# ErickRosete/tacorl

Hardware: AMD Instinct MI355X
Metric: offline grad-steps/sec (batch=256, 84x84 RGB) (higher is better)
Workload: dtype bf16; 1 GPU; tacorl actor-critic training_step, frozen LMP (BASELINE configs[1]); per_gpu_batch=256, global_batch=256, window=16, image=84x84x3, frames=fp32 CHW (reference batch schema), latent_plan=16, n_action_samples=4, phase=Q (epoch>=bc_epochs), action_decoder_loss=every step (reference behaviour), parallelism=dp1, hip_graph=True, losses_finite=True

## Files before the change

### include/tacorl_hip.h

```cpp
#ifndef TACORL_HIP_H
#define TACORL_HIP_H
#include <stddef.h>
#ifdef __cplusplus
extern "C" {
#endif

typedef void* tacorl_stream_t;

#define TACORL_MAXP 16
enum { TACORL_F32 = 0, TACORL_BF16 = 1 };
enum { TACORL_ACT_NONE = 0, TACORL_ACT_RELU = 1, TACORL_ACT_SILU = 2, TACORL_ACT_TANH = 3 };

int tacorl_hip_version(void);
int tacorl_hip_init(int device);
const char* tacorl_hip_last_error(void);
int tacorl_time_mark(unsigned long long* marks, int slot, tacorl_stream_t stream);
int tacorl_time_spin(unsigned long long* marks, int slot, long ticks, tacorl_stream_t stream);

int tacorl_linear_fwd(int nprob, const float* const* x, int ldx, const float* const* w,
                      const float* const* b, float* const* y, float* const* z, const int* M,
                      int K, int N, int act, int compute_dtype, tacorl_stream_t stream);
size_t tacorl_linear_add_fwd_ws_bytes(int nprob, const int* M, int K, int N);
int tacorl_linear_add_fwd(int nprob, const float* const* x, int ldx, const float* const* w,
                          const float* const* b, const float* const* addend, int ld_add, float* const* y,
// ... 294 lines not shown
                      float* dq1, float* dq2, float grad_scale, float* logs, tacorl_stream_t stream);
int tacorl_actor_head_bwd(const float* head, int ld_head, const float* eps, const float* logp,
                          const float* g_act1, const float* g_act2, int ld_g, const float* value,
                          int ld_value, const int* grip_idx, const float* log_alpha, float grad_scale,
                          float* d_head, int B, int Ac, int has_grip, float* logs, tacorl_stream_t stream);
int tacorl_tanh_normal_nll(const float* head, int ld_head, const float* target, int ld_target, int M, int Ac,
                           int has_grip, float grad_scale, float* d_head, float* loss_out, tacorl_stream_t stream);

size_t tacorl_cql_ws_bytes(int B);
int tacorl_cql_loss(const float* q1, const float* q2, float* dq1, float* dq2, const float* tq1,
                    const float* tq2, const float* logp_cur, const float* logp_nxt, const float* next_logp,
                    const float* reward, const float* done, const float* log_alpha,
                    const float* log_alpha_prime, int B, int n, int A, float discount, float reward_scale,
                    float temp, float cons_w, float gap, int deterministic_backup, float grad_scale,
                    float* g_log_alpha_prime, float* logs, void* ws, size_t ws_bytes, tacorl_stream_t stream);

size_t tacorl_adam_ws_bytes(long n);
int tacorl_adam_step(float* param, const float* grad, float* m, float* v, long n, float lr,
                     float max_norm, int* step_counter, float* target, float tau, void* ws,
                     size_t ws_bytes, tacorl_stream_t stream);
size_t tacorl_adam_batch_ws_bytes(int nb);
int tacorl_adam_step_batch(int nb, float* const* param, const float* const* grad, float* const* m,
                           float* const* v, const long* n, const float* lr, const float* max_norm,
                           int* const* step_counter, float* const* target, const float* tau, void* ws,
                           size_t ws_bytes, tacorl_stream_t stream);
int tacorl_adam_step_batch_mirror(int nb, float* const* param, const float* const* grad, float* const* m,
                                  float* const* v, const long* n, const float* lr, const float* max_norm,
                                  int* const* step_counter, float* const* target, const float* tau,
                                  void* const* mirror, void* const* target_mirror, void* ws, size_t ws_bytes,
                                  tacorl_stream_t stream);
// ... 14 lines not shown
```

### tacorl_amd/_lib.py

```python
import ctypes as C
import os

HERE = os.path.dirname(os.path.abspath(__file__))
LIB_PATH = os.environ.get("TACORL_HIP_LIB") or os.path.join(HERE, "lib", "libtacorl_hip.so")

F32, BF16 = 0, 1
ACT_NONE, ACT_RELU, ACT_SILU, ACT_TANH = 0, 1, 2, 3
MAXP = 16

LOG_SLOTS = [
    "alpha_loss", "alpha", "actor_loss", "bellman_q1_loss", "bellman_q2_loss", "conservative_q1_loss",
    "conservative_q2_loss", "q1_loss", "q2_loss", "alpha_prime", "alpha_prime_loss", "q1_data", "q1_random",
    "q1_policy", "q2_data", "q2_random", "q2_policy", "action_loss",
]

_p, _i, _l, _f, _sz = C.c_void_p, C.c_int, C.c_long, C.c_float, C.c_size_t
_SIGS = {
    "tacorl_hip_version": (_i, []),
    "tacorl_hip_init": (_i, [_i]),
    "tacorl_hip_last_error": (C.c_char_p, []),
    "tacorl_time_mark": (_i, [_p, _i, _p]),
    "tacorl_time_spin": (_i, [_p, _i, _l, _p]),
    "tacorl_linear_fwd": (_i, [_i, _p, _i, _p, _p, _p, _p, _p, _i, _i, _i, _i, _p]),
    "tacorl_linear_add_fwd_ws_bytes": (_sz, [_i, _p, _i, _i]),
# ... 106 lines not shown
    "tacorl_sample_transitions": (_i, [_p, _l, _p, _p, _i, _p, _l, _p, _p, _p, _p, _p, _p, _l, _l, _i, _i, _p, _p, _p, _p, _p, _p]),
    "tacorl_copy_cols": (_i, [_p, _i, _p, _i, _i, _i, _i, _i, _p]),
    "tacorl_copy_cols_batch": (_i, [_i, _p, _p, _p, _p, _p, _p, _p, _p, _p]),
    "tacorl_reduce_rows_mod": (_i, [_p, _i, _p, _i, _i, _i, _i, _p]),
    "tacorl_reduce_rows_mod_batch": (_i, [_i, _p, _i, _p, _i, _i, _i, _i, _p]),
    "tacorl_uniform_actions": (_i, [_p, _p, _i, _i, _i, _i, _p]),
    "tacorl_tanh_normal_sample": (_i, [_p, _i, _p, _p, _i, _p, _i, _p, _p, _i, _i, _i, _p]),
    "tacorl_tanh_normal_sample_batch": (_i, [_i, _p, _i, _p, _p, _p, _p, _i, _p, _p, _p, _i, _i, _p, _p, _i, _i, _i, _p]),
    "tacorl_alpha_loss": (_i, [_p, _i, _p, _f, _f, _p, _p, _p]),
    "tacorl_alpha_loss_step": (_i, [_p, _i, _p, _f, _p, _p, _p, _p, _f, _p, _p]),
    "tacorl_actor_qmin": (_i, [_p, _p, _p, _i, _p, _p, _p, _f, _p, _p]),
    "tacorl_actor_head_bwd": (_i, [_p, _i, _p, _p, _p, _p, _i, _p, _i, _p, _p, _f, _p, _i, _i, _i, _p, _p]),
    "tacorl_tanh_normal_nll": (_i, [_p, _i, _p, _i, _i, _i, _i, _f, _p, _p, _p]),
    "tacorl_cql_ws_bytes": (_sz, [_i]),
    "tacorl_cql_loss": (_i, [_p] * 13 + [_i, _i, _i, _f, _f, _f, _f, _f, _i, _f, _p, _p, _p, _sz, _p]),
    "tacorl_adam_ws_bytes": (_sz, [_l]),
    "tacorl_adam_step": (_i, [_p, _p, _p, _p, _l, _f, _f, _p, _p, _f, _p, _sz, _p]),
    "tacorl_adam_batch_ws_bytes": (_sz, [_i]),
    "tacorl_adam_step_batch": (_i, [_i, _p, _p, _p, _p, _p, _p, _p, _p, _p, _p, _p, _sz, _p]),
    "tacorl_adam_step_batch_mirror": (_i, [_i, _p, _p, _p, _p, _p, _p, _p, _p, _p, _p, _p, _p, _p, _sz, _p]),
    "tacorl_cem_supported": (_i, [_i, _i, _i, _i, _i, _i]),
    "tacorl_cem_ws_bytes": (_sz, [_i, _i, _i, _i, _i, _i, _i]),
    "tacorl_cem_refine": (_i, [_i, _i, _p, _p, _p, _p, _p, _p, _i, _i, _i, _i, _i, _i, _i, _f, _f, _f, _i, _i, _p, _p, _p, _p, _p,
                               _p, _sz, _p]),
}

_lib = None


class TacorlHipError(RuntimeError):
# ... 71 lines not shown
```

### tacorl_amd/csrc/dense_ops.hip

```cpp
#include <stdio.h>
#include <stdlib.h>
#include <string.h>

#include <type_traits>

#include "../../include/tacorl_hip.h"
#include "enc_bwd_fused.h"
#include "mlp_fused.h"
#include "functors.h"

static thread_local char g_err[256] = "";
#define FAIL(code, ...)                        \
  do {                                         \
    snprintf(g_err, sizeof(g_err), __VA_ARGS__); \
    return (code);                             \
  } while (0)
#define CHECK(x)            \
  do {                      \
    int _r = (x);           \
    if (_r != TACORL_OK) return _r; \
  } while (0)

extern "C" const char* tacorl_hip_last_error(void) { return g_err; }
extern "C" int tacorl_hip_version(void) { return 1; }
// ... 998 lines not shown
  for (int p = 0; p < nprob; p++) {
    long z1[MLP_MAXL], y1[MLP_MAXL];
    tacorl_mlp_act_layout(M[p], L, dims, acts, z1, y1);
    const int b = (lean && mlp_big_prob_ok(M[p], L, dims, acts)) ? 1 : 0, q = n[b]++;
    gm[b][q] = p;
    xs[b][q] = x ? x[p] : nullptr; ps[b][q] = params[p]; pb[b][q] = params_bf16[p]; as[b][q] = act[p]; Ms[b][q] = M[p];
    for (int l = 0; l < L; l++) {
      if (b) { ybf[q * MF_MAXL + l] = y1[l]; sbf[q * MF_MAXL + l] = z1[l]; }
      else {
        zo[q * MF_MAXL + l] = z1[l];
        yo[q * MF_MAXL + l] = (lean && l + 1 < L && z1[l] >= 0) ? -1 : y1[l];
      }
    }
    if (b) yout[q] = y1[L - 1];
  }
  if (n[1]) {
    const int rc = mlp_big_fwd(n[1], xs[1], ldx, ps[1], pb[1], as[1], Ms[1], L, dims, acts, ybf, sbf, yout, wo, bo, (hipStream_t)stream, gather, gm[1]);
    if (rc != TACORL_OK) FAIL(rc, "mlp_fwd_fused: many-row launch failed (%d)", rc);
  }
  if (n[0]) {
    const int rc = mlp_fused_fwd(n[0], xs[0], ldx, ps[0], pb[0], as[0], Ms[0], L, dims, acts, zo, yo, wo, bo, (hipStream_t)stream, gather, gm[0]);
    if (rc != TACORL_OK) FAIL(rc, "mlp_fwd_fused: launch failed (%d)", rc);
  }
  return TACORL_OK;
}
extern "C" int tacorl_mlp_fwd_fused(int nprob, const float* const* x, int ldx, const float* const* params,
                                    const void* const* params_bf16, float* const* act, const int* M, int L,
                                    const int* dims, const int* acts, int lean, tacorl_stream_t stream) {
  return mlp_fwd_fused_impl(nprob, x, ldx, params, params_bf16, act, M, L, dims, acts, lean, stream, nullptr);
}
// ... 310 lines not shown
```

### tacorl_amd/csrc/mlp_fused.h

```cpp
#pragma once
#include <hip/hip_runtime.h>

#define MF_MAXP 8
#define MF_MAXL 4
#define MF_MAXSEG 4

struct MlpXGather {
  const float* ptr[MF_MAXP][MF_MAXSEG];
  int ld[MF_MAXP][MF_MAXSEG], c0[MF_MAXP][MF_MAXSEG], mod[MF_MAXP][MF_MAXSEG];
  int nseg[MF_MAXP];
  float* xw[MF_MAXP];
};

bool mlp_fused_fwd_ok(int nprob, int L, const int* dims, int ldx);
int mlp_fused_fwd(int nprob, const float* const* x, int ldx, const float* const* params, const void* const* params_bf16,
                  float* const* act,
                  const int* M, int L, const int* dims, const int* acts, const long* zoff, const long* yoff,
                  const long* woff, const long* boff, hipStream_t st, const MlpXGather* gather = nullptr,
                  const int* gmap = nullptr);

bool mlp_fused_bwd_ok(int nprob, int L, const int* dims, int ldo, int ldd);
size_t mlp_fused_wt_elems(int L, const int* dims, long* wtoff);
int mlp_fused_bwd(int nprob, const float* const* params, const float* const* act, const float* const* d_out, int ldo,
                  float* const* dz, float* const* d_x, int ldd, void* const* wt, const int* M, int L, const int* dims,
// ... 1 lines not shown
bool prep_deferring();
int prep_defer_bf16(const float* src, void* dst, long count, hipStream_t st);

bool mlp_fused_wgrad_ok(int nprob, int L, const int* dims);
size_t mlp_fused_wgrad_slab_floats(int nprob, const int* M, int L, const int* dims);
int mlp_fused_wgrad(int nprob, const float* const* x, int ldx, const float* const* act, const float* const* d_out, int ldo,
                    const float* const* dz, float* const* grads, float* slab, const int* M, int L, const int* dims,
                    const long* yoff, const long* dzoff, const long* woff, const long* boff, int accumulate, hipStream_t st,
                    const int* acts = nullptr);

bool mlp_big_prob_ok(int M, int L, const int* dims, const int* acts);
int mlp_big_fwd(int nprob, const float* const* x, int ldx, const float* const* params, const void* const* params_bf16,
                float* const* act, const int* M, int L, const int* dims, const int* acts, const long* ybf, const long* sbf,
                const long* yout, const long* woff, const long* boff, hipStream_t st, const MlpXGather* gather = nullptr,
                const int* gmap = nullptr);
int mlp_big_bwd(int nprob, const float* const* act, const float* const* d_out, int ldo, float* const* dz, float* const* d_x,
                int ldd, void* const* wt, const int* M, int L, const int* dims, const long* sbf, const long* dzoff,
                hipStream_t st);
size_t mlp_big_wgrad_slab_floats(int nprob, const int* M, int L, const int* dims);
size_t mlp_big_xb_bytes(int M);
int mlp_fused_wgrad_big(int nprob, const float* const* x, int ldx, const float* const* act, const float* const* d_out, int ldo,
                        const float* const* dz, float* const* grads, float* slab, void* const* xb, const int* M, int L,
                        const int* dims, const long* ybf, const long* dzoff, const long* woff, const long* boff, int accumulate,
                        hipStream_t st, size_t slab_floats);
```

### tacorl_amd/csrc/mlp_fused.hip

```cpp
#include "mlp_fused.h"

#include <stdlib.h>

#include "common.h"

namespace {

constexpr int BMF = 32;
constexpr int MTF = BMF / 16;
constexpr int XP = 272;
constexpr int MAXD = 256;
constexpr int MF_NT = 1024, MF_CW = MAXD / (MF_NT / 64), MF_NTW = MF_CW / 16;

struct MlpXSeg { const float* p; int ld, c0, mod, pad; };
struct MlpFwdArgs {
  MlpXSeg seg[MF_MAXP][MF_MAXSEG];
  int nseg[MF_MAXP];
  float* xw[MF_MAXP];
  const float* x[MF_MAXP];
  const float* params[MF_MAXP];
  const __bf16* pbf[MF_MAXP];
  float* act[MF_MAXP];
  int M[MF_MAXP];
  long zoff[MF_MAXP][MF_MAXL], yoff[MF_MAXP][MF_MAXL];
// ... 32 lines not shown
      const __bf16* q = W + (long)n * K;
#pragma unroll
      for (int e = 0; e < 8; e++)
        if (k + e < K) v[e] = q[k + e];
    }
    return v;
  }
  const bool on = n < N && k < K;
  const __bf16* q = W + (long)(on ? n : 0) * K + (on ? k : 0);
  const bf16x4 lo = *reinterpret_cast<const bf16x4*>(q), hi = *reinterpret_cast<const bf16x4*>(q + 4);
  const __bf16 z = (__bf16)0.f;
  return on ? bf16x8{lo[0], lo[1], lo[2], lo[3], hi[0], hi[1], hi[2], hi[3]} : bf16x8{z, z, z, z, z, z, z, z};
}

template <int BMF_>
__device__ __forceinline__ void mlp_fused_fwd_body(const MlpFwdArgs& a) {
  constexpr int BMF = BMF_, MTF = BMF_ / 16;
  extern __shared__ __attribute__((aligned(16))) unsigned char smem[];
  __bf16* X = reinterpret_cast<__bf16*>(smem);
  const int p = blockIdx.y, m0 = blockIdx.x * BMF, M = a.M[p];
  if (m0 >= M) return;
  const int tid = threadIdx.x, lane = tid & 63, w = tid >> 6, i = lane & 15, g = lane >> 4;
  const int n0 = MF_CW * w;
  bf16x8 B[8][MF_NTW];
  auto load_layer = [&](int l) {
    const int K = a.dims[l], N = a.dims[l + 1];
    const __bf16* Wb = a.pbf[p] + a.woff[l];
#pragma unroll
    for (int ks = 0; ks < 8; ks++)
#pragma unroll
      for (int nt = 0; nt < MF_NTW; nt++) B[ks][nt] = load_w(Wb, K, N, n0 + 16 * nt + i, 32 * ks + 8 * g);
  };
  if (n0 < a.dims[1]) load_layer(0);
  for (int e = tid; e < 2 * BMF * XP / 8; e += MF_NT) reinterpret_cast<f32x4*>(X)[e] = f32x4{0.f, 0.f, 0.f, 0.f};
  __syncthreads();
// ... 113 lines not shown
#pragma unroll
              for (int r = 0; r < 4; r++)
                if (col + r < N) { if (zb) zb[o + r] = z[r]; if (yb) yb[o + r] = y[r]; }
            }
          }
          *reinterpret_cast<bf16x4*>(xout + row * XP + col) = bf16x4{(__bf16)y[0], (__bf16)y[1], (__bf16)y[2], (__bf16)y[3]};
        }
      }
    }
    lds_barrier();
    cur ^= 1;
  }
}

__global__ __launch_bounds__(MF_NT) __attribute__((amdgpu_waves_per_eu(5, 8))) void mlp_fused_fwd_kernel(MlpFwdArgs a) {
  mlp_fused_fwd_body<32>(a);
}
__global__ __launch_bounds__(MF_NT) void mlp_fused_fwd_big_kernel(MlpFwdArgs a) { mlp_fused_fwd_body<128>(a); }

struct MlpBwdArgs {
  const float* d_out[MF_MAXP];
  const float* act[MF_MAXP];
  const __bf16* wt[MF_MAXP];
  float* dz[MF_MAXP];
  float* d_x[MF_MAXP];
  int M[MF_MAXP];
  long srcoff[MF_MAXP][MF_MAXL];
  long dzoff[MF_MAXP][MF_MAXL];
  long wtoff[MF_MAXL];
  int dims[MF_MAXL + 1], acts[MF_MAXL];
  int L, ldo, ldd;
};

// ... 405 lines not shown
  float* xw[MF_MAXP];
  const float* x[MF_MAXP];
  const float* params[MF_MAXP];
  const __bf16* pbf[MF_MAXP];
  float* act[MF_MAXP];
  int M[MF_MAXP];
  long ybf[MF_MAXP][MF_MAXL], sbf[MF_MAXP][MF_MAXL];
  long yout[MF_MAXP];
  long woff[MF_MAXL], boff[MF_MAXL];
  int dims[MF_MAXL + 1], acts[MF_MAXL];
  int L, ldx;
  int dbg;
};

template <int BMF_>
__device__ __forceinline__ void mlp_big_fwd_body(const MlpBigFwdArgs& a) {
  constexpr int BMF = BMF_, MTF = BMF / 16;
  extern __shared__ __attribute__((aligned(16))) unsigned char smem[];
  __bf16* X = reinterpret_cast<__bf16*>(smem);
  const int p = blockIdx.y, m0 = blockIdx.x * BMF, M = a.M[p];
  const int Mp = (M + 63) & ~63;
  if (m0 >= Mp) return;
  const int tid = threadIdx.x, lane = tid & 63, w = tid >> 6, i = lane & 15, g = lane >> 4;
  const int n0 = MF_CW * w;
#ifdef MLP_STAMPS
  const bool stamp_on = blockIdx.x == 300 && p == 0 && tid == 0;
#endif
  MLP_STAMP(0, 0);
  const int K0 = a.dims[0], c8 = (K0 + 7) / 8;
  f32x4 xr[2][2];
  const float* x = a.x[p];
  const int ns = a.nseg[p];
#pragma unroll
  for (int u = 0; u < 2; u++) {
    const int c = tid + u * MF_NT, row = c / c8, k = (c - row * c8) * 8;
    const bool ok = c < BMF * c8 && m0 + row < M;
    if (ns > 0) {
      int sg = 0;
#pragma unroll
      for (int t = 1; t < MF_MAXSEG; t++) sg = (t < ns && k >= a.seg[p][t].c0) ? t : sg;
      const MlpXSeg s = a.seg[p][sg];
// ... 147 lines not shown
          const __bf16 z0 = (__bf16)0.f;
          bf16x8 yv = {z0, z0, z0, z0, z0, z0, z0, z0}, sv = yv;
          if (m0 + row < M) {
            yv = *reinterpret_cast<const bf16x8*>(xout + row * XP + k);
            sv = *reinterpret_cast<const bf16x8*>(reinterpret_cast<const __bf16*>(sb) + row * XP + k);
          }
          *reinterpret_cast<bf16x8*>(y16 + (long)(m0 + row) * N + k) = yv;
          *reinterpret_cast<bf16x8*>(s16 + (long)(m0 + row) * N + k) = sv;
        }
      }
    }
    MLP_STAMP(0, 8 * l + 7);
    cur ^= 1;
  }
}
__global__ __launch_bounds__(MF_NT) void mlp_big_fwd_kernel(MlpBigFwdArgs a) { mlp_big_fwd_body<128>(a); }
__global__ __launch_bounds__(MF_NT) __attribute__((amdgpu_waves_per_eu(5, 8))) void mlp_mid_fwd_kernel(MlpBigFwdArgs a) { mlp_big_fwd_body<32>(a); }

constexpr int PF_NT = 512, PF_BM = 64, PF_MT = PF_BM / 16, PF_K0S = 3;
constexpr int PF_XB = 2 * PF_BM * XP * 2, PF_SB = PF_BM * XP * 2, PF_W0B = 8 * PF_K0S * 2 * 1024, PF_MISC = 8192;
constexpr int PF_LDS = PF_XB + PF_SB + PF_W0B + PF_MISC;
static_assert(PF_LDS <= 160 * 1024, "persistent forward: LDS");
typedef unsigned int pf_u32x4 __attribute__((ext_vector_type(4)));
typedef _Float16 f16x8 __attribute__((ext_vector_type(8)));

template <int NH>
__global__ __launch_bounds__(PF_NT) void mlp_pers_fwd_kernel(MlpBigFwdArgs a) {
  extern __shared__ __attribute__((aligned(16))) unsigned char smem[];
  __bf16* X = reinterpret_cast<__bf16*>(smem);
  _Float16* S = reinterpret_cast<_Float16*>(smem + PF_XB);
  pf_u32x4* W0 = reinterpret_cast<pf_u32x4*>(smem + PF_XB + PF_SB);
  float* BI = reinterpret_cast<float*>(smem + PF_XB + PF_SB + PF_W0B);
// ... 920 lines not shown
static int mlp_set_gather(Args& a, int p, int q, const MlpXGather* gather, int K0) {
  const int ns = gather ? gather->nseg[q] : 0;
  if (ns < 0 || ns > MF_MAXSEG) return TACORL_EINVAL;
  a.nseg[p] = ns;
  a.xw[p] = ns ? gather->xw[q] : nullptr;
  if ((uintptr_t)a.xw[p] & 15) return TACORL_EINVAL;
  for (int t = 0; t < ns; t++) {
    const int c0 = gather->c0[q][t], ld = gather->ld[q][t];
    if (((uintptr_t)gather->ptr[q][t] & 15) || !gather->ptr[q][t] || ld % 4 || c0 % 8 || (t == 0 ? c0 != 0 : c0 <= gather->c0[q][t - 1]) ||
        c0 >= K0 || gather->mod[q][t] < 0)
      return TACORL_EINVAL;
    a.seg[p][t] = MlpXSeg{gather->ptr[q][t], ld, c0, gather->mod[q][t], 0};
  }
  return TACORL_OK;
}
int mlp_big_fwd(int nprob, const float* const* x, int ldx, const float* const* params, const void* const* params_bf16,
                float* const* act, const int* M, int L, const int* dims, const int* acts, const long* ybf, const long* sbf,
                const long* yout, const long* woff, const long* boff, hipStream_t st, const MlpXGather* gather, const int* gmap) {
  MlpBigFwdArgs a{};
  int maxM = 0;
  for (int p = 0; p < nprob; p++) {
    if (mlp_set_gather(a, p, gmap ? gmap[p] : p, gather, dims[0]) != TACORL_OK) return TACORL_EINVAL;
    if ((!a.nseg[p] && ((uintptr_t)x[p] & 15)) || ((uintptr_t)params[p] & 15) || ((uintptr_t)params_bf16[p] & 7) || ((uintptr_t)act[p] & 15)) return TACORL_EINVAL;
    a.x[p] = x[p]; a.params[p] = params[p]; a.pbf[p] = (const __bf16*)params_bf16[p]; a.act[p] = act[p]; a.M[p] = M[p];
    for (int l = 0; l < L; l++) { a.ybf[p][l] = ybf[p * MF_MAXL + l]; a.sbf[p][l] = sbf[p * MF_MAXL + l]; }
    a.yout[p] = yout[p];
    maxM = M[p] > maxM ? M[p] : maxM;
  }
  for (int l = 0; l < L; l++) {
    if (woff[l] % 4) return TACORL_EINVAL;
    a.woff[l] = woff[l]; a.boff[l] = boff[l]; a.dims[l] = dims[l]; a.acts[l] = acts[l];
  }
  a.dims[L] = dims[L]; a.L = L; a.ldx = ldx;
  if (maxM == 0) return TACORL_OK;
  constexpr size_t lds = (size_t)2 * 128 * XP * 2, lds_mid = (size_t)2 * 32 * XP * 2;
  static int once = (hipFuncSetAttribute(reinterpret_cast<const void*>(mlp_big_fwd_kernel),
                                         hipFuncAttributeMaxDynamicSharedMemorySize, (int)lds) == hipSuccess &&
                     hipFuncSetAttribute(reinterpret_cast<const void*>(mlp_mid_fwd_kernel),
                                         hipFuncAttributeMaxDynamicSharedMemorySize, (int)lds_mid) == hipSuccess) ? 0 : -1;
  if (once) return TACORL_ELAUNCH;
  const int maxMp = (maxM + 63) & ~63;
  {
    const char* pe = getenv("TACORL_MLP_PERS");
    bool pers = mlp_rows_huge(maxM) && (pe ? atoi(pe) : 1) && (L == 3 || L == 4) && dims[0] <= 32 * PF_K0S && dims[L] <= 4;
    for (int l = 0; l + 1 < L && pers; l++) pers = acts[l] == ACT_SILU && dims[l + 1] == 256;
    if (pers) {
      static int once_p = (hipFuncSetAttribute(reinterpret_cast<const void*>(mlp_pers_fwd_kernel<1>),
                                               hipFuncAttributeMaxDynamicSharedMemorySize, PF_LDS) == hipSuccess &&
// ... 194 lines not shown
  if (once) return TACORL_ELAUNCH;
  if (maxM >= MLP_BIG_ROWS)
    hipLaunchKernelGGL(mlp_fused_bwd_big_kernel, dim3((maxM + 63) / 64, nprob), dim3(MF_NT), lds_big, st, a);
  else
    hipLaunchKernelGGL(mlp_fused_bwd_kernel, dim3((maxM + BMF - 1) / BMF, nprob), dim3(MF_NT), lds, st, a);
  return hipGetLastError() == hipSuccess ? TACORL_OK : TACORL_ELAUNCH;
}

bool mlp_fused_fwd_ok(int nprob, int L, const int* dims, int ldx) {
  if (nprob < 1 || nprob > MF_MAXP || L < 1 || L > MF_MAXL || ldx % 4) return false;
  for (int l = 0; l < L; l++)
    if ((l > 0 && dims[l] % 8) || dims[l] > MAXD || dims[l] < 8) return false;
  return dims[L] >= 1 && dims[L] <= MAXD;
}

int mlp_fused_fwd(int nprob, const float* const* x, int ldx, const float* const* params, const void* const* params_bf16,
                  float* const* act,
                  const int* M, int L, const int* dims, const int* acts, const long* zoff, const long* yoff,
                  const long* woff, const long* boff, hipStream_t st, const MlpXGather* gather, const int* gmap) {
  MlpFwdArgs a{};
  int maxM = 0;
  for (int p = 0; p < nprob; p++) {
    if (mlp_set_gather(a, p, gmap ? gmap[p] : p, gather, dims[0]) != TACORL_OK) return TACORL_EINVAL;
    const int ns = a.nseg[p];
    if (ns) {
      if ((uintptr_t)params[p] & 15) return TACORL_EINVAL;
    } else if (((uintptr_t)x[p] & 15) || ((uintptr_t)params[p] & 15)) return TACORL_EINVAL;
    if ((uintptr_t)params_bf16[p] & 7) return TACORL_EINVAL;
    a.x[p] = x[p]; a.params[p] = params[p]; a.pbf[p] = (const __bf16*)params_bf16[p]; a.act[p] = act[p]; a.M[p] = M[p];
    for (int l = 0; l < L; l++) { a.zoff[p][l] = zoff[p * MF_MAXL + l]; a.yoff[p][l] = yoff[p * MF_MAXL + l]; }
    maxM = M[p] > maxM ? M[p] : maxM;
  }
  for (int l = 0; l < L; l++) {
    if (woff[l] % 4) return TACORL_EINVAL;
    a.woff[l] = woff[l]; a.boff[l] = boff[l]; a.dims[l] = dims[l]; a.acts[l] = acts[l];
  }
  a.dims[L] = dims[L]; a.L = L; a.ldx = ldx;
  if (maxM == 0) return TACORL_OK;
  constexpr size_t lds = (size_t)2 * BMF * XP * 2, lds_big = (size_t)2 * 128 * XP * 2;
  static int once = (hipFuncSetAttribute(reinterpret_cast<const void*>(mlp_fused_fwd_kernel),
                                         hipFuncAttributeMaxDynamicSharedMemorySize, (int)lds) == hipSuccess &&
                     hipFuncSetAttribute(reinterpret_cast<const void*>(mlp_fused_fwd_big_kernel),
                                         hipFuncAttributeMaxDynamicSharedMemorySize, (int)lds_big) == hipSuccess) ? 0 : -1;
  if (once) return TACORL_ELAUNCH;
  if (maxM >= MLP_BIG_ROWS)
    hipLaunchKernelGGL(mlp_fused_fwd_big_kernel, dim3((maxM + 127) / 128, nprob), dim3(MF_NT), lds_big, st, a);
  else
    hipLaunchKernelGGL(mlp_fused_fwd_kernel, dim3((maxM + BMF - 1) / BMF, nprob), dim3(MF_NT), lds, st, a);
  return hipGetLastError() == hipSuccess ? TACORL_OK : TACORL_ELAUNCH;
}
```

### tacorl_amd/csrc/rl_ops.hip

```cpp
#include <stdio.h>

#include "../../include/tacorl_hip.h"
#include "common.h"

#define LAUNCH_OK() (hipGetLastError() == hipSuccess ? TACORL_OK : TACORL_ELAUNCH)

__device__ __forceinline__ float softplusf(float x) {
  return x > 20.f ? x : log1pf(expf(x));
}
__device__ __forceinline__ float block_sum_256(float v, float* sh) {
  v = wave_sum(v);
  __syncthreads();
  if ((threadIdx.x & 63) == 0) sh[threadIdx.x >> 6] = v;
  __syncthreads();
  return sh[0] + sh[1] + sh[2] + sh[3];
}

template <typename OutT>
__global__ void pack_images_kernel(const float* __restrict__ src, long img_pitch, int src_nchw,
                                   OutT* __restrict__ dst, int n, int C, int HW) {
  const long total = (long)n * HW;
  for (long i = (long)blockIdx.x * blockDim.x + threadIdx.x; i < total; i += (long)gridDim.x * blockDim.x) {
    const long img = i / HW;
    const int px = (int)(i - img * HW);
// ... 794 lines not shown
    logs[LG_ALPHA_P] = alpha_p;
    logs[LG_ALPHA_P_LOSS] = (-cons[0] - cons[1]) * 0.5f;
    g_log_alpha_prime[0] = (ea >= 0.f && ea <= 1000000.f) ? -0.5f * raw * ea * a.grad_scale : 0.f;
  }
  logs[LG_BELL1] = bell[0]; logs[LG_BELL2] = bell[1];
  logs[LG_CONS1] = cons[0]; logs[LG_CONS2] = cons[1];
  logs[LG_Q1LOSS] = bell[0] + cons[0]; logs[LG_Q2LOSS] = bell[1] + cons[1];
  logs[LG_Q1_DATA] = tot[CP_D1] / B; logs[LG_Q2_DATA] = tot[CP_D2] / B;
  logs[LG_Q1_RAND] = tot[CP_R1] / nB; logs[LG_Q2_RAND] = tot[CP_R2] / nB;
  logs[LG_Q1_POL] = tot[CP_P1] / nB; logs[LG_Q2_POL] = tot[CP_P2] / nB;
}
extern "C" size_t tacorl_cql_ws_bytes(int B) {
  const int blocks = (B + 3) / 4 > 256 ? 256 : (B + 3) / 4;
  return (size_t)blocks * 4 * CP_N * sizeof(float);
}
extern "C" int tacorl_cql_loss(const float* q1, const float* q2, float* dq1, float* dq2, const float* tq1,
                               const float* tq2, const float* logp_cur, const float* logp_nxt,
                               const float* next_logp, const float* reward, const float* done,
                               const float* log_alpha, const float* log_alpha_prime, int B, int n, int A,
                               float discount, float reward_scale, float temp, float cons_w, float gap,
                               int deterministic_backup, float grad_scale, float* g_log_alpha_prime, float* logs,
                               void* ws, size_t ws_bytes, tacorl_stream_t stream) {
  if (3 * n > 128 || n < 1) return TACORL_EINVAL;
  if (ws_bytes < tacorl_cql_ws_bytes(B)) return TACORL_ENOMEM;
  CqlArgs a{};
  a.q[0] = q1; a.q[1] = q2; a.dq[0] = dq1; a.dq[1] = dq2; a.tq[0] = tq1; a.tq[1] = tq2;
  a.logp_cur = logp_cur; a.logp_nxt = logp_nxt; a.next_logp = next_logp; a.reward = reward; a.done = done;
  a.log_alpha = log_alpha; a.log_alpha_prime = log_alpha_prime; a.partial = (float*)ws;
  a.B = B; a.n = n; a.A = A; a.discount = discount; a.reward_scale = reward_scale; a.temp = temp; a.cons_w = cons_w;
  a.gap = gap; a.grad_scale = grad_scale; a.deterministic_backup = deterministic_backup;
  const int blocks = (B + 3) / 4 > 256 ? 256 : (B + 3) / 4;
  hipLaunchKernelGGL(cql_loss_kernel, dim3(blocks), dim3(256), 0, (hipStream_t)stream, a);
  hipLaunchKernelGGL(cql_finish_kernel, dim3(1), dim3(256), 0, (hipStream_t)stream, a, blocks * 4, g_log_alpha_prime,
                     logs);
  return LAUNCH_OK();
}

__global__ __launch_bounds__(256) void sqnorm_partial_kernel(const float* __restrict__ g, long n, float* partial) {
  __shared__ float sh[4];
  float s = 0.f;
  for (long i = (long)blockIdx.x * 256 + threadIdx.x; i < n; i += (long)gridDim.x * 256) s += g[i] * g[i];
  s = block_sum_256(s, sh);
  if (threadIdx.x == 0) partial[blockIdx.x] = s;
}
__global__ __launch_bounds__(256) void adam_kernel(float* __restrict__ p, const float* __restrict__ g,
                                                   float* __restrict__ m, float* __restrict__ v, long n, float lr,
                                                   const float* partial, int nparts, float max_norm,
                                                   int* step_counter, float* __restrict__ target, float tau) {
  __shared__ float sh[4];
  float coef = 1.f;
// ... 180 lines not shown
```

### tacorl_amd/csrc/rnn_ops.hip

```cpp
#include <hip/hip_runtime.h>
#include <stdint.h>
#include <stdio.h>
#include <stdlib.h>

#include "../../include/tacorl_hip.h"
#include "common.h"

namespace {

constexpr int RB_K = 128;
constexpr int ROW_BYTES = RB_K * 2;

struct RnnArgs {
  const __bf16* x;
  const __bf16* w;
  const float* bias;
  const float* addend;
  const float* mask_src;
  float* y;
  __bf16* yb;
  int M, K, N, ld_add, act;
  const __bf16* x2;
  const float* addend2;
  float* y2;
// ... 16 lines not shown
    const int jx = blockIdx.x;
    mt = jx % MT; ntile = (jx / MT) % NT; prob = jx / (MT * NT);
  } else {
    const int xcd = blockIdx.x & 7, jx = blockIdx.x >> 3, rx = jx / MT;
    mt = jx % MT; ntile = xcd * NTX + rx % NTX; prob = rx / NTX;
    if (ntile >= NT) return;
  }
  const RnnArgs a = ab.p[prob];
  constexpr int STAGE_BYTES = (RB_M + RB_N) * ROW_BYTES;
  constexpr int DMA_PER_WAVE = (RB_M + RB_N) / 4 / NW;
  constexpr int MI = RB_M / (16 * NW), NI = RB_N / 16;
  static_assert((RB_M + RB_N) % (4 * NW) == 0 && RB_M % (16 * NW) == 0 && RB_N % 16 == 0, "tile shape");
  extern __shared__ __attribute__((aligned(16))) unsigned char lds[];
  const int tid = threadIdx.x, lane = tid & 63, w = tid >> 6, i = lane & 15, g = lane >> 4;
  const int m0 = mt * RB_M, n0 = ntile * RB_N;
  const int nkm = a.K / RB_K, nk = nkm + (a.x_ext ? 1 : 0), mtot = a.M + a.M2;
  const long ldx = a.ldx ? a.ldx : a.K, ldy = a.ldy ? a.ldy : a.N;

  auto issue = [&](int kt, int slot) {
    unsigned char* base = lds + slot * STAGE_BYTES;
#pragma unroll
    for (int q = 0; q < DMA_PER_WAVE; q++) {
      const int row4 = (w + NW * q) * 4;
      const int r = row4 + (lane >> 4), cpos = lane & 15, c = cpos ^ (r & 15);
      const int xm = m0 + r < mtot ? m0 + r : mtot - 1;
      const __bf16* src;
      if (kt < nkm) {
        const __bf16* xrow = xm < a.M ? a.x + xm * ldx : a.x2 + (long)(xm - a.M) * a.K;
        src = (r < RB_M ? xrow : a.w + (long)(n0 + r - RB_M) * a.K) + kt * RB_K + c * 8;
      } else {
        const __bf16* xrow = xm < a.M ? a.x_ext + (long)xm * RB_K : a.x2_ext + (long)(xm - a.M) * RB_K;
// ... 421 lines not shown
  return hipGetLastError() == hipSuccess ? TACORL_OK : TACORL_ELAUNCH;
}

static int rnn_fwd_batch(int nprob, const void* const* x_bf16, const void* const* w_bf16, const float* const* bias,
                         const float* const* addend, int ld_add, float* const* y, void* const* y_bf16, int M, int K, int N,
                         const int* acts, const void* const* x2_bf16, const float* const* addend2, float* const* y2,
                         void* const* y2_bf16, int M2, tacorl_stream_t stream, const void* const* x_ext = nullptr,
                         const void* const* x2_ext = nullptr, const void* const* w_ext = nullptr, const float* const* bias2 = nullptr) {
  if (nprob < 1 || nprob > RNN_MAXP || !tacorl_rnn_linear_supported(M, K, N) || ld_add % 4 || M2 < 0) return TACORL_EINVAL;
  if (M2 > 0 && (!x2_bf16 || !y2)) return TACORL_EINVAL;
  RnnBatch ab{};
  for (int p = 0; p < nprob; p++) {
    const float* ad = addend ? addend[p] : nullptr;
    const float* bi = bias ? bias[p] : nullptr;
    void* yb = y_bf16 ? y_bf16[p] : nullptr;
    if (((uintptr_t)x_bf16[p] | (uintptr_t)w_bf16[p] | (uintptr_t)y[p] | (uintptr_t)bi | (uintptr_t)ad) & 15) return TACORL_EINVAL;
    if ((uintptr_t)yb & 7) return TACORL_EINVAL;
    ab.p[p] = RnnArgs{(const __bf16*)x_bf16[p], (const __bf16*)w_bf16[p], bi, ad, nullptr, y[p], (__bf16*)yb, M, K, N, ld_add, acts[p]};
    if (x_ext && x_ext[p]) {
      if (!w_ext || !w_ext[p] || (((uintptr_t)x_ext[p] | (uintptr_t)w_ext[p] | (uintptr_t)(bias2 ? bias2[p] : nullptr)) & 15)) return TACORL_EINVAL;
      if (M2 > 0 && x2_bf16[p] && (!x2_ext || !x2_ext[p] || ((uintptr_t)x2_ext[p] & 15))) return TACORL_EINVAL;
      ab.p[p].x_ext = (const __bf16*)x_ext[p]; ab.p[p].w_ext = (const __bf16*)w_ext[p];
      ab.p[p].x2_ext = M2 > 0 && x2_ext ? (const __bf16*)x2_ext[p] : nullptr;
      ab.p[p].bias2 = bias2 ? bias2[p] : nullptr;
    }
    if (M2 > 0 && x2_bf16[p]) {
      const float* ad2 = addend2 ? addend2[p] : nullptr;
      void* yb2 = y2_bf16 ? y2_bf16[p] : nullptr;
      if (!y2[p] || (((uintptr_t)x2_bf16[p] | (uintptr_t)y2[p] | (uintptr_t)ad2) & 15) || ((uintptr_t)yb2 & 7)) return TACORL_EINVAL;
      ab.p[p].x2 = (const __bf16*)x2_bf16[p]; ab.p[p].addend2 = ad2; ab.p[p].y2 = y2[p]; ab.p[p].yb2 = (__bf16*)yb2;
// ... 70 lines not shown
```

### tacorl_amd/networks/action_decoder.py

```python
import ctypes as C

import torch

from .. import ops
from .._lib import ACT_NONE, ACT_RELU, call, ptr
from ..blocks import TensorBlock


RNN_MAXP = 4


class ActionDecoderLogistic:
    def __init__(self, device, state_dim=32, goal_dim=32, latent_plan_dim=16, hidden_size=256, out_features=7,
                 act_max_bound=(1.0,) * 7, act_min_bound=(-1.0,) * 7, gripper_alpha=1.0, policy_rnn_dropout_p=0.0,
                 num_layers=2, rnn_model="rnn_decoder", discrete_gripper=True, include_goal=False, num_classes=10,
                 n_mixtures=10, **unused):
        if rnn_model != "rnn_decoder" or not discrete_gripper or include_goal or policy_rnn_dropout_p != 0.0:
            raise NotImplementedError("only the configured decoder (relu nn.RNN, discrete gripper, no goal) is in scope")
        if any(abs(b - 1.0) > 0 for b in act_max_bound) or any(abs(b + 1.0) > 0 for b in act_min_bound):
            raise NotImplementedError("action bounds other than +-1 (config/networks/action_decoder/logistic.yaml)")
        self.dev, self.P, self.E, self.hidden, self.L = device, latent_plan_dim, state_dim, hidden_size, num_layers
        self.Da, self.K, self.num_classes, self.gripper_alpha = out_features - 1, n_mixtures, num_classes, gripper_alpha
        self.include_goal = include_goal
        H, In, DK = hidden_size, state_dim + latent_plan_dim, (out_features - 1) * n_mixtures
# ... 218 lines not shown
                     ptr(self.xin[0]), B, T, Tm, self.P, self.E, H, ops.stream())
            else:
                self._lin(x, K, blk.p("rnn.weight_ih_l0"), blk.p("rnn.bias_ih_l0"), self.xin[0], R, K, H, ACT_NONE, compute)
            L = self.L
            assert twin is None or (proj_fused and twin.shape == (B, Tm)), "twin pass: twin_ok() / twin_state(B, Tm)"
            hbp = lambda l, t, o=self: C.c_void_p(o.hb[l].data_ptr() + 2 * t * B * H)
            xbp = lambda t, o=self: C.c_void_p(o.xb_seq.data_ptr() + 2 * t * B * 128)
            for s_ in range(Tm + 2 * (L - 1)):
                xs, wt, bs, ad, ys, yb, ac = [], [], [], [], [], [], []
                x2, ad2, y2, yb2 = [], [], [], []
                xe, xe2, we, b2 = [], [], [], []
                for l in range(L):
                    t = s_ - 2 * l
                    if 0 <= t < Tm:
                        ext = ring and l == 0
                        xs.append(ptr(self.h0b) if t == 0 else hbp(l, t - 1)); wt.append(ptr(self.whb[l]))
                        bs.append(blk.p(f"rnn.bias_hh_l{l}")); ad.append(None if ext else at(self.xin[l], t * B * H))
                        ys.append(at(self.h[l], t * B * H)); yb.append(hbp(l, t)); ac.append(ACT_RELU)
                        xe.append(xbp(t) if ext else None); we.append(ptr(self.wih0_b) if ext else None)
                        b2.append(blk.p("rnn.bias_ih_l0") if ext else None)
                        if twin is not None:
                            x2.append(ptr(self.h0b) if t == 0 else hbp(l, t - 1, twin))
                            ad2.append(None if ext else at(twin.xin[l], t * B * H))
                            y2.append(at(twin.h[l], t * B * H)); yb2.append(hbp(l, t, twin))
                            xe2.append(xbp(t, twin) if ext else None)
                    t = s_ - 2 * l + 1
                    if l >= 1 and 0 <= t < Tm:
                        xs.append(hbp(l - 1, t)); wt.append(ptr(self.wib[l])); bs.append(blk.p(f"rnn.bias_ih_l{l}"))
                        ad.append(None); ys.append(at(self.xin[l], t * B * H)); yb.append(None); ac.append(ACT_NONE)
                        xe.append(None); we.append(None); b2.append(None)
                        if twin is not None:
# ... 272 lines not shown
```

Measured before the change: 1233 grad-steps/s.

## Fuse big and small MLP forward groups into one paired launch; skip zero-state RNN GEMM

Adds a paired MLP forward kernel that runs the many-row and few-row problem groups in a single launch, dispatching by blockIdx.y, in place of two back-to-back launches. It also lets the RNN step at t=0 skip the hidden-state matmul against the all-zero initial state by passing a null input. It splits the CQL loss into separately callable row and finish entry points, though nothing shown calls them yet. The paired kernel uses the larger LDS size and the mid (32-row) tile for the big group, which may lower per-block efficiency for that group.

```diff
diff --git a/include/tacorl_hip.h b/include/tacorl_hip.h
--- a/include/tacorl_hip.h
+++ b/include/tacorl_hip.h
@@ -332,6 +332,18 @@
                     const float* log_alpha_prime, int B, int n, int A, float discount, float reward_scale,
                     float temp, float cons_w, float gap, int deterministic_backup, float grad_scale,
                     float* g_log_alpha_prime, float* logs, void* ws, size_t ws_bytes, tacorl_stream_t stream);
+int tacorl_cql_loss_rows(const float* q1, const float* q2, float* dq1, float* dq2, const float* tq1,
+                    const float* tq2, const float* logp_cur, const float* logp_nxt, const float* next_logp,
+                    const float* reward, const float* done, const float* log_alpha,
+                    const float* log_alpha_prime, int B, int n, int A, float discount, float reward_scale,
+                    float temp, float cons_w, float gap, int deterministic_backup, float grad_scale,
+                    float* g_log_alpha_prime, float* logs, void* ws, size_t ws_bytes, tacorl_stream_t stream);
+int tacorl_cql_loss_finish(const float* q1, const float* q2, float* dq1, float* dq2, const float* tq1,
+                    const float* tq2, const float* logp_cur, const float* logp_nxt, const float* next_logp,
+                    const float* reward, const float* done, const float* log_alpha,
+                    const float* log_alpha_prime, int B, int n, int A, float discount, float reward_scale,
+                    float temp, float cons_w, float gap, int deterministic_backup, float grad_scale,
+                    float* g_log_alpha_prime, float* logs, void* ws, size_t ws_bytes, tacorl_stream_t stream);
 
 size_t tacorl_adam_ws_bytes(long n);
 int tacorl_adam_step(float* param, const float* grad, float* m, float* v, long n, float lr,
diff --git a/tacorl_amd/_lib.py b/tacorl_amd/_lib.py
--- a/tacorl_amd/_lib.py
+++ b/tacorl_amd/_lib.py
@@ -144,6 +144,8 @@
     "tacorl_tanh_normal_nll": (_i, [_p, _i, _p, _i, _i, _i, _i, _f, _p, _p, _p]),
     "tacorl_cql_ws_bytes": (_sz, [_i]),
     "tacorl_cql_loss": (_i, [_p] * 13 + [_i, _i, _i, _f, _f, _f, _f, _f, _i, _f, _p, _p, _p, _sz, _p]),
+    "tacorl_cql_loss_rows": (_i, [_p] * 13 + [_i, _i, _i, _f, _f, _f, _f, _f, _i, _f, _p, _p, _p, _sz, _p]),
+    "tacorl_cql_loss_finish": (_i, [_p] * 13 + [_i, _i, _i, _f, _f, _f, _f, _f, _i, _f, _p, _p, _p, _sz, _p]),
     "tacorl_adam_ws_bytes": (_sz, [_l]),
     "tacorl_adam_step": (_i, [_p, _p, _p, _p, _l, _f, _f, _p, _p, _f, _p, _sz, _p]),
     "tacorl_adam_batch_ws_bytes": (_sz, [_i]),
diff --git a/tacorl_amd/csrc/dense_ops.hip b/tacorl_amd/csrc/dense_ops.hip
--- a/tacorl_amd/csrc/dense_ops.hip
+++ b/tacorl_amd/csrc/dense_ops.hip
@@ -1036,6 +1036,13 @@
     }
     if (b) yout[q] = y1[L - 1];
   }
+  const char* pe = getenv("TACORL_MLP_PAIR");
+  if ((pe ? atoi(pe) : 1) && mlp_pair_fwd_ok(n[1], Ms[1], n[0], Ms[0])) {
+    const int rc = mlp_pair_fwd(n[1], xs[1], ps[1], pb[1], as[1], Ms[1], ybf, sbf, yout, gm[1], n[0], xs[0], ps[0], pb[0], as[0], Ms[0],
+                                zo, yo, gm[0], ldx, L, dims, acts, wo, bo, (hipStream_t)stream, gather);
+    if (rc != TACORL_OK) FAIL(rc, "mlp_fwd_fused: paired launch failed (%d)", rc);
+    return TACORL_OK;
+  }
   if (n[1]) {
     const int rc = mlp_big_fwd(n[1], xs[1], ldx, ps[1], pb[1], as[1], Ms[1], L, dims, acts, ybf, sbf, yout, wo, bo, (hipStream_t)stream, gather, gm[1]);
     if (rc != TACORL_OK) FAIL(rc, "mlp_fwd_fused: many-row launch failed (%d)", rc);
diff --git a/tacorl_amd/csrc/mlp_fused.h b/tacorl_amd/csrc/mlp_fused.h
--- a/tacorl_amd/csrc/mlp_fused.h
+++ b/tacorl_amd/csrc/mlp_fused.h
@@ -39,6 +39,12 @@
                 float* const* act, const int* M, int L, const int* dims, const int* acts, const long* ybf, const long* sbf,
                 const long* yout, const long* woff, const long* boff, hipStream_t st, const MlpXGather* gather = nullptr,
                 const int* gmap = nullptr);
+bool mlp_pair_fwd_ok(int nbig, const int* Mbig, int nsmall, const int* Msmall);
+int mlp_pair_fwd(int nbig, const float* const* xb, const float* const* pb, const void* const* pbb, float* const* ab, const int* Mb,
+                 const long* ybf, const long* sbf, const long* yout, const int* gmb, int nsmall, const float* const* xs,
+                 const float* const* ps, const void* const* pbs, float* const* as, const int* Ms, const long* zoff, const long* yoff,
+                 const int* gms, int ldx, int L, const int* dims, const int* acts, const long* woff, const long* boff, hipStream_t st,
+                 const MlpXGather* gather = nullptr);
 int mlp_big_bwd(int nprob, const float* const* act, const float* const* d_out, int ldo, float* const* dz, float* const* d_x,
                 int ldd, void* const* wt, const int* M, int L, const int* dims, const long* sbf, const long* dzoff,
                 hipStream_t st);
diff --git a/tacorl_amd/csrc/mlp_fused.hip b/tacorl_amd/csrc/mlp_fused.hip
--- a/tacorl_amd/csrc/mlp_fused.hip
+++ b/tacorl_amd/csrc/mlp_fused.hip
@@ -70,11 +70,11 @@
 }
 
 template <int BMF_>
-__device__ __forceinline__ void mlp_fused_fwd_body(const MlpFwdArgs& a) {
+__device__ __forceinline__ void mlp_fused_fwd_body(const MlpFwdArgs& a, const int bx, const int p) {
   constexpr int BMF = BMF_, MTF = BMF_ / 16;
   extern __shared__ __attribute__((aligned(16))) unsigned char smem[];
   __bf16* X = reinterpret_cast<__bf16*>(smem);
-  const int p = blockIdx.y, m0 = blockIdx.x * BMF, M = a.M[p];
+  const int m0 = bx * BMF, M = a.M[p];
   if (m0 >= M) return;
   const int tid = threadIdx.x, lane = tid & 63, w = tid >> 6, i = lane & 15, g = lane >> 4;
   const int n0 = MF_CW * w;
@@ -218,9 +218,9 @@
 }
 
 __global__ __launch_bounds__(MF_NT) __attribute__((amdgpu_waves_per_eu(5, 8))) void mlp_fused_fwd_kernel(MlpFwdArgs a) {
-  mlp_fused_fwd_body<32>(a);
-}
-__global__ __launch_bounds__(MF_NT) void mlp_fused_fwd_big_kernel(MlpFwdArgs a) { mlp_fused_fwd_body<128>(a); }
+  mlp_fused_fwd_body<32>(a, blockIdx.x, blockIdx.y);
+}
+__global__ __launch_bounds__(MF_NT) void mlp_fused_fwd_big_kernel(MlpFwdArgs a) { mlp_fused_fwd_body<128>(a, blockIdx.x, blockIdx.y); }
 
 struct MlpBwdArgs {
   const float* d_out[MF_MAXP];
@@ -656,17 +656,17 @@
 };
 
 template <int BMF_>
-__device__ __forceinline__ void mlp_big_fwd_body(const MlpBigFwdArgs& a) {
+__device__ __forceinline__ void mlp_big_fwd_body(const MlpBigFwdArgs& a, const int bx, const int p) {
   constexpr int BMF = BMF_, MTF = BMF / 16;
   extern __shared__ __attribute__((aligned(16))) unsigned char smem[];
   __bf16* X = reinterpret_cast<__bf16*>(smem);
-  const int p = blockIdx.y, m0 = blockIdx.x * BMF, M = a.M[p];
+  const int m0 = bx * BMF, M = a.M[p];
   const int Mp = (M + 63) & ~63;
   if (m0 >= Mp) return;
   const int tid = threadIdx.x, lane = tid & 63, w = tid >> 6, i = lane & 15, g = lane >> 4;
   const int n0 = MF_CW * w;
 #ifdef MLP_STAMPS
-  const bool stamp_on = blockIdx.x == 300 && p == 0 && tid == 0;
+  const bool stamp_on = bx == 300 && p == 0 && tid == 0;
 #endif
   MLP_STAMP(0, 0);
   const int K0 = a.dims[0], c8 = (K0 + 7) / 8;
@@ -844,8 +844,16 @@
     cur ^= 1;
   }
 }
-__global__ __launch_bounds__(MF_NT) void mlp_big_fwd_kernel(MlpBigFwdArgs a) { mlp_big_fwd_body<128>(a); }
-__global__ __launch_bounds__(MF_NT) __attribute__((amdgpu_waves_per_eu(5, 8))) void mlp_mid_fwd_kernel(MlpBigFwdArgs a) { mlp_big_fwd_body<32>(a); }
+__global__ __launch_bounds__(MF_NT) void mlp_big_fwd_kernel(MlpBigFwdArgs a) { mlp_big_fwd_body<128>(a, blockIdx.x, blockIdx.y); }
+__global__ __launch_bounds__(MF_NT) __attribute__((amdgpu_waves_per_eu(5, 8))) void mlp_mid_fwd_kernel(MlpBigFwdArgs a) {
+  mlp_big_fwd_body<32>(a, blockIdx.x, blockIdx.y);
+}
+static_assert(sizeof(MlpBigFwdArgs) + sizeof(MlpFwdArgs) + sizeof(int) <= 4096, "mlp_pair_fwd_kernel: kernel-argument limit");
+__global__ __launch_bounds__(MF_NT) __attribute__((amdgpu_waves_per_eu(5, 8))) void mlp_pair_fwd_kernel(MlpBigFwdArgs ab, MlpFwdArgs as, int nbig) {
+  const int by = blockIdx.y;
+  if (by < nbig) mlp_big_fwd_body<32>(ab, blockIdx.x, by);
+  else mlp_fused_fwd_body<32>(as, blockIdx.x, by - nbig);
+}
 
 constexpr int PF_NT = 512, PF_BM = 64, PF_MT = PF_BM / 16, PF_K0S = 3;
 constexpr int PF_XB = 2 * PF_BM * XP * 2, PF_SB = PF_BM * XP * 2, PF_W0B = 8 * PF_K0S * 2 * 1024, PF_MISC = 8192;
@@ -1796,11 +1804,12 @@
   }
   return TACORL_OK;
 }
-int mlp_big_fwd(int nprob, const float* const* x, int ldx, const float* const* params, const void* const* params_bf16,
-                float* const* act, const int* M, int L, const int* dims, const int* acts, const long* ybf, const long* sbf,
-                const long* yout, const long* woff, const long* boff, hipStream_t st, const MlpXGather* gather, const int* gmap) {
-  MlpBigFwdArgs a{};
-  int maxM = 0;
+static int mlp_big_fwd_fill(MlpBigFwdArgs& a, int& maxM, int nprob, const float* const* x, int ldx, const float* const* params,
+                            const void* const* params_bf16, float* const* act, const int* M, int L, const int* dims, const int* acts,
+                            const long* ybf, const long* sbf, const long* yout, const long* woff, const long* boff,
+                            const MlpXGather* gather, const int* gmap) {
+  a = MlpBigFwdArgs{};
+  maxM = 0;
   for (int p = 0; p < nprob; p++) {
     if (mlp_set_gather(a, p, gmap ? gmap[p] : p, gather, dims[0]) != TACORL_OK) return TACORL_EINVAL;
     if ((!a.nseg[p] && ((uintptr_t)x[p] & 15)) || ((uintptr_t)params[p] & 15) || ((uintptr_t)params_bf16[p] & 7) || ((uintptr_t)act[p] & 15)) return TACORL_EINVAL;
@@ -1814,6 +1823,15 @@
     a.woff[l] = woff[l]; a.boff[l] = boff[l]; a.dims[l] = dims[l]; a.acts[l] = acts[l];
   }
   a.dims[L] = dims[L]; a.L = L; a.ldx = ldx;
+  return TACORL_OK;
+}
+int mlp_big_fwd(int nprob, const float* const* x, int ldx, const float* const* params, const void* const* params_bf16,
+                float* const* act, const int* M, int L, const int* dims, const int* acts, const long* ybf, const long* sbf,
+                const long* yout, const long* woff, const long* boff, hipStream_t st, const MlpXGather* gather, const int* gmap) {
+  MlpBigFwdArgs a;
+  int maxM;
+  const int rcf = mlp_big_fwd_fill(a, maxM, nprob, x, ldx, params, params_bf16, act, M, L, dims, acts, ybf, sbf, yout, woff, boff, gather, gmap);
+  if (rcf != TACORL_OK) return rcf;
   if (maxM == 0) return TACORL_OK;
   constexpr size_t lds = (size_t)2 * 128 * XP * 2, lds_mid = (size_t)2 * 32 * XP * 2;
   static int once = (hipFuncSetAttribute(reinterpret_cast<const void*>(mlp_big_fwd_kernel),
@@ -2038,12 +2056,12 @@
   return dims[L] >= 1 && dims[L] <= MAXD;
 }
 
-int mlp_fused_fwd(int nprob, const float* const* x, int ldx, const float* const* params, const void* const* params_bf16,
-                  float* const* act,
-                  const int* M, int L, const int* dims, const int* acts, const long* zoff, const long* yoff,
-                  const long* woff, const long* boff, hipStream_t st, const MlpXGather* gather, const int* gmap) {
-  MlpFwdArgs a{};
-  int maxM = 0;
+static int mlp_fused_fwd_fill(MlpFwdArgs& a, int& maxM, int nprob, const float* const* x, int ldx, const float* const* params,
+                              const void* const* params_bf16, float* const* act, const int* M, int L, const int* dims,
+                              const int* acts, const long* zoff, const long* yoff, const long* woff, const long* boff,
+                              const MlpXGather* gather, const int* gmap) {
+  a = MlpFwdArgs{};
+  maxM = 0;
   for (int p = 0; p < nprob; p++) {
     if (mlp_set_gather(a, p, gmap ? gmap[p] : p, gather, dims[0]) != TACORL_OK) return TACORL_EINVAL;
     const int ns = a.nseg[p];
@@ -2060,6 +2078,16 @@
     a.woff[l] = woff[l]; a.boff[l] = boff[l]; a.dims[l] = dims[l]; a.acts[l] = acts[l];
   }
   a.dims[L] = dims[L]; a.L = L; a.ldx = ldx;
+  return TACORL_OK;
+}
+int mlp_fused_fwd(int nprob, const float* const* x, int ldx, const float* const* params, const void* const* params_bf16,
+                  float* const* act,
+                  const int* M, int L, const int* dims, const int* acts, const long* zoff, const long* yoff,
+                  const long* woff, const long* boff, hipStream_t st, const MlpXGather* gather, const int* gmap) {
+  MlpFwdArgs a;
+  int maxM;
+  const int rcf = mlp_fused_fwd_fill(a, maxM, nprob, x, ldx, params, params_bf16, act, M, L, dims, acts, zoff, yoff, woff, boff, gather, gmap);
+  if (rcf != TACORL_OK) return rcf;
   if (maxM == 0) return TACORL_OK;
   constexpr size_t lds = (size_t)2 * BMF * XP * 2, lds_big = (size_t)2 * 128 * XP * 2;
   static int once = (hipFuncSetAttribute(reinterpret_cast<const void*>(mlp_fused_fwd_kernel),
@@ -2073,3 +2101,31 @@
     hipLaunchKernelGGL(mlp_fused_fwd_kernel, dim3((maxM + BMF - 1) / BMF, nprob), dim3(MF_NT), lds, st, a);
   return hipGetLastError() == hipSuccess ? TACORL_OK : TACORL_ELAUNCH;
 }
+
+bool mlp_pair_fwd_ok(int nbig, const int* Mbig, int nsmall, const int* Msmall) {
+  if (nbig < 1 || nsmall < 1 || nbig + nsmall > MF_MAXP) return false;
+  int mb = 0, ms = 0;
+  for (int p = 0; p < nbig; p++) mb = Mbig[p] > mb ? Mbig[p] : mb;
+  for (int p = 0; p < nsmall; p++) ms = Msmall[p] > ms ? Msmall[p] : ms;
+  return mb > 0 && ms > 0 && !mlp_rows_huge(mb) && ms < MLP_BIG_ROWS;
+}
+int mlp_pair_fwd(int nbig, const float* const* xb, const float* const* pb, const void* const* pbb, float* const* ab, const int* Mb,
+                 const long* ybf, const long* sbf, const long* yout, const int* gmb, int nsmall, const float* const* xs,
+                 const float* const* ps, const void* const* pbs, float* const* as, const int* Ms, const long* zoff, const long* yoff,
+                 const int* gms, int ldx, int L, const int* dims, const int* acts, const long* woff, const long* boff, hipStream_t st,
+                 const MlpXGather* gather) {
+  if (!mlp_pair_fwd_ok(nbig, Mb, nsmall, Ms)) return TACORL_EINVAL;
+  MlpBigFwdArgs big;
+  MlpFwdArgs sm;
+  int maxb, maxs;
+  int rc = mlp_big_fwd_fill(big, maxb, nbig, xb, ldx, pb, pbb, ab, Mb, L, dims, acts, ybf, sbf, yout, woff, boff, gather, gmb);
+  if (rc == TACORL_OK) rc = mlp_fused_fwd_fill(sm, maxs, nsmall, xs, ldx, ps, pbs, as, Ms, L, dims, acts, zoff, yoff, woff, boff, gather, gms);
+  if (rc != TACORL_OK) return rc;
+  constexpr size_t lds_mid = (size_t)2 * 32 * XP * 2, lds_small = (size_t)2 * BMF * XP * 2, lds = lds_mid > lds_small ? lds_mid : lds_small;
+  static int once = hipFuncSetAttribute(reinterpret_cast<const void*>(mlp_pair_fwd_kernel), hipFuncAttributeMaxDynamicSharedMemorySize,
+                                        (int)lds) == hipSuccess ? 0 : -1;
+  if (once) return TACORL_ELAUNCH;
+  const int gb = ((maxb + 63) & ~63) / 32, gs = (maxs + BMF - 1) / BMF;
+  hipLaunchKernelGGL(mlp_pair_fwd_kernel, dim3(gb > gs ? gb : gs, nbig + nsmall), dim3(MF_NT), lds, st, big, sm, nbig);
+  return hipGetLastError() == hipSuccess ? TACORL_OK : TACORL_ELAUNCH;
+}
diff --git a/tacorl_amd/csrc/rl_ops.hip b/tacorl_amd/csrc/rl_ops.hip
--- a/tacorl_amd/csrc/rl_ops.hip
+++ b/tacorl_amd/csrc/rl_ops.hip
@@ -832,13 +832,12 @@
   const int blocks = (B + 3) / 4 > 256 ? 256 : (B + 3) / 4;
   return (size_t)blocks * 4 * CP_N * sizeof(float);
 }
-extern "C" int tacorl_cql_loss(const float* q1, const float* q2, float* dq1, float* dq2, const float* tq1,
-                               const float* tq2, const float* logp_cur, const float* logp_nxt,
-                               const float* next_logp, const float* reward, const float* done,
-                               const float* log_alpha, const float* log_alpha_prime, int B, int n, int A,
-                               float discount, float reward_scale, float temp, float cons_w, float gap,
-                               int deterministic_backup, float grad_scale, float* g_log_alpha_prime, float* logs,
-                               void* ws, size_t ws_bytes, tacorl_stream_t stream) {
+static int cql_loss_launch(int parts, const float* q1, const float* q2, float* dq1, float* dq2, const float* tq1, const float* tq2,
+                           const float* logp_cur, const float* logp_nxt, const float* next_logp, const float* reward,
+                           const float* done, const float* log_alpha, const float* log_alpha_prime, int B, int n, int A,
+                           float discount, float reward_scale, float temp, float cons_w, float gap, int deterministic_backup,
+                           float grad_scale, float* g_log_alpha_prime, float* logs, void* ws, size_t ws_bytes,
+                           tacorl_stream_t stream) {
   if (3 * n > 128 || n < 1) return TACORL_EINVAL;
   if (ws_bytes < tacorl_cql_ws_bytes(B)) return TACORL_ENOMEM;
   CqlArgs a{};
@@ -848,10 +847,43 @@
   a.B = B; a.n = n; a.A = A; a.discount = discount; a.reward_scale = reward_scale; a.temp = temp; a.cons_w = cons_w;
   a.gap = gap; a.grad_scale = grad_scale; a.deterministic_backup = deterministic_backup;
   const int blocks = (B + 3) / 4 > 256 ? 256 : (B + 3) / 4;
-  hipLaunchKernelGGL(cql_loss_kernel, dim3(blocks), dim3(256), 0, (hipStream_t)stream, a);
-  hipLaunchKernelGGL(cql_finish_kernel, dim3(1), dim3(256), 0, (hipStream_t)stream, a, blocks * 4, g_log_alpha_prime,
-                     logs);
-  return LAUNCH_OK();
+  if (parts & 1) hipLaunchKernelGGL(cql_loss_kernel, dim3(blocks), dim3(256), 0, (hipStream_t)stream, a);
+  if (parts & 2)
+    hipLaunchKernelGGL(cql_finish_kernel, dim3(1), dim3(256), 0, (hipStream_t)stream, a, blocks * 4, g_log_alpha_prime, logs);
+  return LAUNCH_OK();
+}
+extern "C" int tacorl_cql_loss(const float* q1, const float* q2, float* dq1, float* dq2, const float* tq1,
+                               const float* tq2, const float* logp_cur, const float* logp_nxt,
+                               const float* next_logp, const float* reward, const float* done,
+                               const float* log_alpha, const float* log_alpha_prime, int B, int n, int A,
+                               float discount, float reward_scale, float temp, float cons_w, float gap,
+                               int deterministic_backup, float grad_scale, float* g_log_alpha_prime, float* logs,
+                               void* ws, size_t ws_bytes, tacorl_stream_t stream) {
+  return cql_loss_launch(3, q1, q2, dq1, dq2, tq1, tq2, logp_cur, logp_nxt, next_logp, reward, done, log_alpha, log_alpha_prime, B, n,
+                         A, discount, reward_scale, temp, cons_w, gap, deterministic_backup, grad_scale, g_log_alpha_prime, logs, ws,
+                         ws_bytes, stream);
+}
+extern "C" int tacorl_cql_loss_rows(const float* q1, const float* q2, float* dq1, float* dq2, const float* tq1,
+                                    const float* tq2, const float* logp_cur, const float* logp_nxt,
+                                    const float* next_logp, const float* reward, const float* done,
+                                    const float* log_alpha, const float* log_alpha_prime, int B, int n, int A,
+                                    float discount, float reward_scale, float temp, float cons_w, float gap,
+                                    int deterministic_backup, float grad_scale, float* g_log_alpha_prime, float* logs,
+                                    void* ws, size_t ws_bytes, tacorl_stream_t stream) {
+  return cql_loss_launch(1, q1, q2, dq1, dq2, tq1, tq2, logp_cur, logp_nxt, next_logp, reward, done, log_alpha, log_alpha_prime, B, n,
+                         A, discount, reward_scale, temp, cons_w, gap, deterministic_backup, grad_scale, g_log_alpha_prime, logs, ws,
+                         ws_bytes, stream);
+}
+extern "C" int tacorl_cql_loss_finish(const float* q1, const float* q2, float* dq1, float* dq2, const float* tq1,
+                                      const float* tq2, const float* logp_cur, const float* logp_nxt,
+                                      const float* next_logp, const float* reward, const float* done,
+                                      const float* log_alpha, const float* log_alpha_prime, int B, int n, int A,
+                                      float discount, float reward_scale, float temp, float cons_w, float gap,
+                                      int deterministic_backup, float grad_scale, float* g_log_alpha_prime, float* logs,
+                                      void* ws, size_t ws_bytes, tacorl_stream_t stream) {
+  return cql_loss_launch(2, q1, q2, dq1, dq2, tq1, tq2, logp_cur, logp_nxt, next_logp, reward, done, log_alpha, log_alpha_prime, B, n,
+                         A, discount, reward_scale, temp, cons_w, gap, deterministic_backup, grad_scale, g_log_alpha_prime, logs, ws,
+                         ws_bytes, stream);
 }
 
 __global__ __launch_bounds__(256) void sqnorm_partial_kernel(const float* __restrict__ g, long n, float* partial) {
diff --git a/tacorl_amd/csrc/rnn_ops.hip b/tacorl_amd/csrc/rnn_ops.hip
--- a/tacorl_amd/csrc/rnn_ops.hip
+++ b/tacorl_amd/csrc/rnn_ops.hip
@@ -54,7 +54,7 @@
   extern __shared__ __attribute__((aligned(16))) unsigned char lds[];
   const int tid = threadIdx.x, lane = tid & 63, w = tid >> 6, i = lane & 15, g = lane >> 4;
   const int m0 = mt * RB_M, n0 = ntile * RB_N;
-  const int nkm = a.K / RB_K, nk = nkm + (a.x_ext ? 1 : 0), mtot = a.M + a.M2;
+  const int nkm = a.x ? a.K / RB_K : 0, nk = nkm + (a.x_ext ? 1 : 0), mtot = a.M + a.M2;
   const long ldx = a.ldx ? a.ldx : a.K, ldy = a.ldy ? a.ldy : a.N;
 
   auto issue = [&](int kt, int slot) {
@@ -506,6 +506,7 @@
     const float* ad = addend ? addend[p] : nullptr;
     const float* bi = bias ? bias[p] : nullptr;
     void* yb = y_bf16 ? y_bf16[p] : nullptr;
+    if (!w_bf16[p] || !y[p]) return TACORL_EINVAL;
     if (((uintptr_t)x_bf16[p] | (uintptr_t)w_bf16[p] | (uintptr_t)y[p] | (uintptr_t)bi | (uintptr_t)ad) & 15) return TACORL_EINVAL;
     if ((uintptr_t)yb & 7) return TACORL_EINVAL;
     ab.p[p] = RnnArgs{(const __bf16*)x_bf16[p], (const __bf16*)w_bf16[p], bi, ad, nullptr, y[p], (__bf16*)yb, M, K, N, ld_add, acts[p]};
diff --git a/tacorl_amd/networks/action_decoder.py b/tacorl_amd/networks/action_decoder.py
--- a/tacorl_amd/networks/action_decoder.py
+++ b/tacorl_amd/networks/action_decoder.py
@@ -256,7 +256,7 @@
                     t = s_ - 2 * l
                     if 0 <= t < Tm:
                         ext = ring and l == 0
-                        xs.append(ptr(self.h0b) if t == 0 else hbp(l, t - 1)); wt.append(ptr(self.whb[l]))
+                        xs.append(None if t == 0 else hbp(l, t - 1)); wt.append(ptr(self.whb[l]))
                         bs.append(blk.p(f"rnn.bias_hh_l{l}")); ad.append(None if ext else at(self.xin[l], t * B * H))
                         ys.append(at(self.h[l], t * B * H)); yb.append(hbp(l, t)); ac.append(ACT_RELU)
                         xe.append(xbp(t) if ext else None); we.append(ptr(self.wih0_b) if ext else None)
```

New measurement: 1242 grad-steps/s, median of 5. No clear change (+0.7%).
